# MIT-SPARK/Kimera-Semantics

Measured on NVIDIA H100. Metric: depth_frames_per_s, higher is better.
Workload: dtype f32

## Files before the change

### kimera_semantics_b200/csrc/ksg_api.cu

```cuda
#include <cuda_runtime.h>
#include <cub/cub.cuh>

#include <algorithm>
#include <climits>
#include <cmath>
#include <cstdio>
#include <cstdlib>
#include <cstring>
#include <memory>
#include <numeric>
#include <string>
#include <type_traits>
#include <unordered_map>
#include <unordered_set>
#include <utility>
#include <vector>

#include "../../include/ksg.h"
#include "ksg_kernels.cuh"
#include "ksg_chain.cuh"
#include "ksg_hot.cuh"
#include "ksg_bundle_order.cuh"
#include "ksg_fast.cuh"
#include "ksg_fast3.cuh"
// ... 154 lines not shown
  int frame_stamp = 0;
  int64_t num_blocks = 0;
  int64_t last_blocks_touched = 0;

  int cap_points = 0;
  float4 *pt_pC = nullptr, *pt_pG = nullptr;
  uint8_t *pt_label = nullptr, *pt_flags = nullptr;
  uint32_t* pt_color = nullptr;
  uint64_t* pt_key = nullptr;
  uint8_t* flags8 = nullptr;
  int* pix_list = nullptr;
  int* point_of_seq = nullptr;
  uint32_t *sq_keys = nullptr, *sq_keys_out = nullptr;
  uint32_t *iota = nullptr;

  int *start_next = nullptr, *start_min = nullptr, *start_max = nullptr;
  uint32_t *start_table = nullptr;
  int *s_base = nullptr, *s_visits = nullptr;
  uint32_t *s_hmin = nullptr, *s_hmax = nullptr;
  uint8_t *clear_ff = nullptr, *clear_00 = nullptr;
  uint64_t set_offset = 0;
  int64_t reset_counter = 0;
  int* cast_seq = nullptr;
  float4* ray_param = nullptr;
  uint8_t *ray_label = nullptr, *ray_flags = nullptr;
  uint32_t* ray_color = nullptr;
  int* nsteps = nullptr;
  RayState* ray_state = nullptr;
  long long* ext_off = nullptr;
  Obs3 o3{};

  uint64_t* ks_sorted = nullptr;
  uint32_t* seq_sorted = nullptr;
  int *bstart = nullptr, *bundle_f = nullptr;
  float *hist = nullptr, *tmp = nullptr, *tmp4 = nullptr;
// ... 27 lines not shown
  uint8_t* cub_temp = nullptr;
  size_t cub_temp_bytes = 0;

  uint8_t* h_stage = nullptr;
  size_t h_stage_bytes = 0;
  uint8_t* d_in = nullptr;
  size_t d_in_bytes = 0;

  uint8_t* d_exp = nullptr;
  size_t d_exp_bytes = 0;
  int* d_exp_slots = nullptr;
  int exp_slots_cap = 0;

  FastCounters* d_fc = nullptr;
  FastCounters* h_fc = nullptr;
  int *blk_cnt = nullptr, *blk_off = nullptr, *warp_cnt = nullptr, *warp_off = nullptr, *seq_of_i = nullptr;
  uint32_t* keys32 = nullptr;
  int *tile_cnt = nullptr, *tile_slot = nullptr;
  TileDesc* tile_list = nullptr;
  FastTile* fast_tiles = nullptr;
  FastItem* fast_items = nullptr;
  int item_cap = 0;
  int solve_grid = 0, group_grid = 0, fast_apply_grid = 0;
  int solve_threads = 0;
  RayRec* rayrec = nullptr;
  int* wl = nullptr;
  int *mixed_list = nullptr, *m_list = nullptr, *blk_run = nullptr;
  VoxelUpdate *d_log_head = nullptr, *h_log_head = nullptr;
  float *d_log_prior = nullptr, *h_log_prior = nullptr;
  int log_cap = 0;
  int64_t merged_log_count = 0;
// ... 77 lines not shown
    why = "unknown merged_bundle_order"; return KSG_ERR_INVALID_ARGUMENT; }
  if (c->hot_voxel_mode < 0 || c->hot_voxel_mode > 2) { why = "unknown hot_voxel_mode"; return KSG_ERR_INVALID_ARGUMENT; }
  return KSG_OK;
}

__global__ void k_iota(uint32_t* p, int n) { const int i = blockIdx.x * blockDim.x + threadIdx.x; if (i < n) p[i] = (uint32_t)i; }

int reset_map(ksg_integrator* h, cudaStream_t s) {
  KSG_CUDA(cudaMemsetAsync(h->map.ht_keys, 0xFF, sizeof(uint64_t) * h->ht_cap, s));
  KSG_CUDA(cudaMemsetAsync(h->map.ht_slot, 0xFF, sizeof(int) * h->ht_cap, s));
  KSG_CUDA(cudaMemsetAsync(h->map.touched_stamp, 0, sizeof(int) * h->ht_cap, s));
  KSG_CUDA(cudaMemsetAsync(h->d_cnt, 0, sizeof(Counters), s));
  if (h->start_table) KSG_CUDA(cudaMemsetAsync(h->start_table, 0xFF, sizeof(uint32_t) * kSetSize, s));
  if (h->o3.table) KSG_CUDA(cudaMemsetAsync(h->o3.table, 0xFF, sizeof(uint32_t) * kSetSize, s));
  if (h->d_fc) KSG_CUDA(cudaMemsetAsync(h->d_fc, 0, sizeof(FastCounters), s));
  if (h->o3.stamp_max) {
    KSG_CUDA(cudaMemsetAsync(h->o3.stamp_max, 0x00, sizeof(uint64_t) * kSetSize, s));
    KSG_CUDA(cudaMemsetAsync(h->o3.stamp_min, 0xFF, sizeof(uint64_t) * kSetSize, s));
  }
  if (h->wl) KSG_CUDA(cudaMemsetAsync(h->wl, 0, sizeof(int) * (size_t)h->cap_points, s));
  if (h->tile_cnt) KSG_CUDA(cudaMemsetAsync(h->tile_cnt, 0, sizeof(int) * (size_t)h->ht_cap * h->dc.tiles_per_block, s));
  h->n_pend = 0; h->n_stash = 0;
  std::memset(h->h_cnt_base, 0, 2 * sizeof(Counters));
  h->set_offset = 0;
  h->reset_counter = 0;
  h->num_blocks = 0;
  h->frame_stamp = 0;
  h->last_blocks_touched = 0;
  h->deferred_status = 0;
  h->merged_log_count = 0;
// ... 174 lines not shown
      h->set_offset = 0;
      KSG_CUDA(cudaMemsetAsync(h->start_table, 0xFF, sizeof(uint32_t) * kSetSize, s));
      KSG_CUDA(cudaMemsetAsync(h->o3.table, 0xFF, sizeof(uint32_t) * kSetSize, s));
    }
  }
  return KSG_OK;
}

int integrate_fast(ksg_integrator* h, const InputDesc& in, const FrameIn& fin, const Xform& T, int cap, cudaStream_t s,
                   ksg_frame_stats* stats) {
  const bool sorted = h->cfg.integration_order_mode == KSG_ORDER_SORTED;
  { const int rcs = advance_sets(h, s); if (rcs) return rcs; }
  FastFrame f{};
  f.cfg = h->dc; f.T = T; f.in = fin; f.in.pix_list = nullptr; f.in.point_of_seq = nullptr;
  f.luts = h->d_luts; f.cnt = h->d_cnt; f.fc = h->d_fc; f.map = h->map;
  f.sb = StartBuf{h->start_next, h->start_min, h->start_max, h->start_table};
  f.set_offset = h->set_offset;
  f.capacity = cap;
  f.n_count_blocks = (cap + kCountBlock - 1) / kCountBlock;
  f.vec_ok = in.d_depth ? (((uintptr_t)in.d_depth % 16 == 0 && (uintptr_t)in.d_label_img % 4 == 0) ? 1 : 0) : 0;
  f.frame_stamp = h->frame_stamp;
  f.profile = (h->profiling && !h->profile_marks_only) ? 1 : 0;
  f.prof_marks = h->profiling ? 1 : 0;
  f.seq_of_i = sorted ? h->seq_of_i : nullptr;
  f.block_cnt = h->blk_cnt; f.block_off = h->blk_off; f.warp_cnt = h->warp_cnt; f.warp_off = h->warp_off;
  f.pt_pG = h->pt_pG; f.pt_label = h->pt_label; f.pt_flags = h->pt_flags; f.pt_color = h->pt_color; f.pt_key = h->pt_key;
  f.cast_flag = h->flags8;
  f.cast_seq = h->cast_seq; f.ray_param = h->ray_param; f.ray_label = h->ray_label; f.ray_flags = h->ray_flags; f.ray_color = h->ray_color;
  f.ray_state = h->ray_state; f.ext_off = h->ext_off;
  f.rec_cap = h->rec_cap; f.keys = h->keys32;
  f.tile_cnt = h->tile_cnt; f.tile_slot = h->tile_slot; f.tile_list = h->tile_list; f.tile_cap = h->tile_cap;
  f.o3 = h->o3;
  f.rayrec = h->rayrec; f.blk_run = h->blk_run;
  f.wl_listed = h->wl;
  f.wl_list[0] = h->wl + h->cap_points; f.wl_list[1] = h->wl + 2 * (size_t)h->cap_points;
  f.log_head = h->d_log_head; f.log_prior = h->d_log_prior; f.log_cap = h->log_cap;
  f.s_base = h->s_base; f.s_hmin = h->s_hmin; f.s_hmax = h->s_hmax; f.s_visits = h->s_visits;
  f.mixed_list = h->mixed_list; f.m_list = h->m_list;

  if (h->profiling) {
    cudaEventRecord(h->ev[0], s);
    KSG_CUDA(cudaMemsetAsync(h->d_fc->dbg, 0, sizeof(h->d_fc->dbg), s));
  }
  KSG_CUDA(cudaMemsetAsync(h->clear_ff, 0xFF, (size_t)kSetSize * 16, s));
  KSG_CUDA(cudaMemsetAsync(h->clear_00, 0x00, (size_t)kSetSize * 13, s));
  KSG_CUDA(cudaMemsetAsync(h->start_min, 0x7F, sizeof(int) * kSetSize, s));
  const int B = 256;
  ++h->n_launches;
  if (in.d_depth) k_fast_count<<<f.n_count_blocks, 256, 0, s>>>(f);
  else k_fast_reset<<<1, 1, 0, s>>>(f);
  if (sorted) {
    h->n_launches += 3;
    if (in.d_depth) k_fast_sqnorm<<<f.n_count_blocks, 256, 0, s>>>(f, h->sq_keys);
    else k_fast_sqnorm_points<<<grid_for(cap, B), B, 0, s>>>(f, h->sq_keys);
    k_fast_pad_keys<<<grid_for(cap, B), B, 0, s>>>(h->d_cnt, cap, h->sq_keys);
    size_t tb = h->cub_temp_bytes;
    ++h->n_libcalls;
    KSG_CUDA(cub::DeviceRadixSort::SortPairs(h->cub_temp, tb, h->sq_keys, h->sq_keys_out, h->iota, (uint32_t*)h->point_of_seq, cap, 0, 32, s));
    k_fast_invert_perm<<<grid_for(cap, B), B, 0, s>>>(h->d_cnt, (const uint32_t*)h->point_of_seq, h->seq_of_i);
  }
  ++h->n_launches;
  if (in.d_depth) k_fast_classify<true><<<f.n_count_blocks, 256, 0, s>>>(f);
  else k_fast_classify<false><<<grid_for(cap, B), B, 0, s>>>(f);
  ++h->n_launches;
  k_fast_start_eval3<<<(cap + kEvalBlock - 1) / kEvalBlock, kEvalBlock, 0, s>>>(f);
  if (h->profiling) cudaEventRecord(h->ev[1], s);
  {
    int max_sweeps = h->cap_points + 2;
    void* args[] = {(void*)&f, (void*)&max_sweeps};
    ++h->n_launches;
    KSG_CUDA(cudaLaunchCooperativeKernel((const void*)k_fast_solve3, dim3(h->solve_grid), dim3(h->solve_threads), args,
                                         (size_t)h->solve_smem, s));
  }
  if (h->profiling) cudaEventRecord(h->ev[2], s);
  {
    ApplySrc src{};
    src.param = h->ray_param; src.label = h->ray_label; src.color = h->ray_color; src.tmp = nullptr;
    h->n_launches += 2;
    k_fast_group<<<h->group_grid, kGroupThreads, 0, s>>>(f, h->fast_items, h->fast_tiles, h->item_cap);
    with_nch(h->apply_nch, [&](auto nch) {
// ... 500 lines not shown
  KSG_CUDA(res.device(&h->map.pool, (size_t)dc.block_stride * (size_t)cfg->max_blocks));
  KSG_CUDA(res.device(&h->d_cnt, 1));
  KSG_CUDA(res.pinned(&h->h_cnt_base, 2));
  std::memset(h->h_cnt_base, 0, 2 * sizeof(Counters));
  h->h_cnt = h->h_cnt_base;
  for (int i = 0; i < 2; ++i) {
    KSG_CUDA(res.event(&h->ev_frame_s[i], cudaEventDisableTiming));
    KSG_CUDA(res.event(&h->ev_copy[i], cudaEventDisableTiming));
    KSG_CUDA(res.event(&h->ev_free[i], cudaEventDisableTiming));
  }
  KSG_CUDA(res.stream(&h->copy_stream));

  const size_t N = (size_t)cfg->max_points;
  h->cap_points = cfg->max_points;
  const bool fast = cfg->integrator_type == KSG_INTEGRATOR_FAST;
  KSG_CUDA(res.device(&h->pt_pC, N)); KSG_CUDA(res.device(&h->pt_pG, N));
  KSG_CUDA(res.device(&h->pt_label, N)); KSG_CUDA(res.device(&h->pt_flags, N));
  KSG_CUDA(res.device(&h->pt_color, N)); KSG_CUDA(res.device(&h->pt_key, N));
  KSG_CUDA(res.device(&h->flags8, 2 * N));
  KSG_CUDA(res.device(&h->pix_list, N));
  KSG_CUDA(res.device(&h->iota, N));
  k_iota<<<grid_for((long long)N, 256), 256>>>(h->iota, (int)N);
  if (cfg->integration_order_mode == KSG_ORDER_SORTED) {
    KSG_CUDA(res.device(&h->point_of_seq, N)); KSG_CUDA(res.device(&h->sq_keys, N)); KSG_CUDA(res.device(&h->sq_keys_out, N));
  }
  KSG_CUDA(res.device(&h->ray_param, N)); KSG_CUDA(res.device(&h->ray_flags, N)); KSG_CUDA(res.device(&h->nsteps, N));
  long long rec_cap = cfg->max_updates > 0 ? cfg->max_updates : (fast ? std::max<long long>(4ll << 20, 64ll * (long long)N) : (64ll << 20));
  if (fast) {
    KSG_CUDA(res.device(&h->start_next, N)); KSG_CUDA(res.device(&h->start_table, kSetSize));
    KSG_CUDA(res.device(&h->clear_ff, (size_t)kSetSize * 16));
    KSG_CUDA(res.device(&h->clear_00, (size_t)kSetSize * 13));
    h->s_base = (int*)h->clear_ff; h->start_max = h->s_base + kSetSize; h->s_hmin = (uint32_t*)(h->start_max + kSetSize);
    h->o3.head = (int*)(h->clear_ff + (size_t)kSetSize * 12);
    h->o3.slot_cnt = (int*)h->clear_00;
    h->s_hmax = (uint32_t*)(h->clear_00 + (size_t)kSetSize * 5); h->s_visits = (int*)(h->clear_00 + (size_t)kSetSize * 9);
    KSG_CUDA(res.device(&h->start_min, kSetSize));
    KSG_CUDA(res.device(&h->cast_seq, N));
    KSG_CUDA(res.device(&h->ray_label, N)); KSG_CUDA(res.device(&h->ray_color, N));
    KSG_CUDA(res.device(&h->ray_state, N)); KSG_CUDA(res.device(&h->ext_off, N * kExtSegs));
    long long ext = cfg->max_ray_steps > 0 ? cfg->max_ray_steps : std::max<long long>(16ll << 20, 64ll * (long long)N);
    Obs3& o3 = h->o3;
    o3.ext_base = (long long)N * kH0;
    o3.cand_cap = o3.ext_base + ext;
    if (o3.cand_cap >= 0x7FFFFFFFll) { o3.cand_cap = 0x7FFFFFFEll; }
    KSG_CUDA(res.device(&o3.cand, (size_t)o3.cand_cap));
    o3.ovf_cap = (int)std::min<long long>(std::max<long long>(1ll << 20, 4ll * (long long)N), 1ll << 28);
    KSG_CUDA(res.device(&o3.ovf, (size_t)o3.ovf_cap));
    KSG_CUDA(res.device(&o3.bkt, (size_t)kSetSize * kBkt3));
    KSG_CUDA(res.device(&o3.stamp_max, 2 * (size_t)kSetSize)); o3.stamp_min = o3.stamp_max + kSetSize;
    KSG_CUDA(res.device(&o3.table, kSetSize));
    KSG_CUDA(res.device(&h->rayrec, N));
// ... 104 lines not shown
    KSG_CUDA(cudaFuncSetAttribute(k_tile_apply<true, 1, true>, cudaFuncAttributeMaxDynamicSharedMemorySize, h->apply_smem));
    rc = for_each_tma_nch([&](auto tma, auto nch) -> int {
      KSG_CUDA(cudaFuncSetAttribute(k_tile_apply<decltype(tma)::value, decltype(nch)::value>, cudaFuncAttributeMaxDynamicSharedMemorySize,
                                    h->apply_smem));
      return KSG_OK;
    });
    if (rc) return rc;
  }
  if (fast) {
    KSG_CUDA(res.device(&h->d_fc, 1));
    KSG_CUDA(cudaMemset(h->d_fc, 0, sizeof(FastCounters)));
    KSG_CUDA(res.pinned(&h->h_fc_base, 2));
    std::memset(h->h_fc_base, 0, 2 * sizeof(FastCounters));
    h->h_fc = h->h_fc_base;
    KSG_CUDA(res.device(&h->blk_cnt, N / kCountBlock + 2)); KSG_CUDA(res.device(&h->blk_off, N / kCountBlock + 2));
    KSG_CUDA(res.device(&h->warp_cnt, N / 32 + 64)); KSG_CUDA(res.device(&h->warp_off, N / 32 + 64));
    if (cfg->integration_order_mode == KSG_ORDER_SORTED) KSG_CUDA(res.device(&h->seq_of_i, N));
    KSG_CUDA(res.device(&h->keys32, (size_t)rec_cap));
    const size_t n_tk = (size_t)h->ht_cap * dc.tiles_per_block;
    KSG_CUDA(res.device(&h->tile_cnt, n_tk)); KSG_CUDA(res.device(&h->tile_slot, n_tk));
    KSG_CUDA(cudaMemset(h->tile_cnt, 0, sizeof(int) * n_tk));
    KSG_CUDA(res.device(&h->tile_list, (size_t)h->tile_cap));
    {
      int per_sm = 0;
      h->solve_threads = knobs.solve_threads;
      h->solve_smem = (int)(sizeof(int) * kSortPerWarp * (h->solve_threads / 32));
      KSG_CUDA(cudaFuncSetAttribute(k_fast_solve3, cudaFuncAttributeMaxDynamicSharedMemorySize, h->solve_smem));
      KSG_CUDA(cudaOccupancyMaxActiveBlocksPerMultiprocessor(&per_sm, k_fast_solve3, h->solve_threads, (size_t)h->solve_smem));
      int coop = 0;
      cudaDeviceGetAttribute(&coop, cudaDevAttrCooperativeLaunch, h->device);
      if (!coop || per_sm <= 0) return h->fail(KSG_ERR_NO_DEVICE, "this device cannot run the fast integrator's observed-set solver "
// ... 1368 lines not shown
```

### kimera_semantics_b200/csrc/ksg_fast.cuh

```cuda
#pragma once
#include "ksg_kernels.cuh"

namespace ksg {

static constexpr int kCountBlock = 1024;
static constexpr int kEvalBlock = 512;
static constexpr int kSolveThreads = 1024;
static constexpr int kFastKeyCap = 4096;
static constexpr int kGroupThreads = 512;
static constexpr int kFastApplyThreads = 256;
static constexpr int kRecVoxMax = 1 << kRecVoxBits;
static constexpr int kTimelineSlots = 64;

struct FastCounters {
  unsigned int ticket_count, ticket_eval;
  unsigned int gridbar;
  int sweep_base;
  int sweeps_last;
  int tile_cursor;
  int n_tile_list;
  int pool_base;
  unsigned long long rec_cursor;
  int ovf_count;
  int n_mixed;
  int m_cursor;
  int log_count;
  int item_cursor;
  int wl_claim[4];
  int wl_count[4];
  long long timeline[kTimelineSlots];
  long long dbg[16];
};

struct TileDesc { uint32_t tk; int n; long long off; };
struct __align__(16) FastTile { long long off; int slot, tile, bx, by, bz, pad; };
struct __align__(16) FastItem { int tile, vox, lo, len; };

struct VoxelUpdate { int bx, by, bz; uint32_t lin_label; float dist, wgt; uint32_t rgba, srgba; };

struct StartBuf {
  int* next;
  int* smin;
  int* smax;
  const uint32_t* table;
};

struct Cand;
struct OvfEnt;
struct RayRec;
struct Obs3 {
  Cand* cand;
  long long ext_base, cand_cap;
  int* slot_cnt;
  uint64_t* bkt;
  int* head;
  OvfEnt* ovf;
  int ovf_cap;
  uint64_t* stamp_max;
  uint64_t* stamp_min;
// ... 6 lines not shown
  FrameIn in;
  const Luts* luts;
  Counters* cnt;
  FastCounters* fc;
  MapRef map;
  StartBuf sb;
  uint64_t set_offset;
  int capacity;
  int n_count_blocks;
  int vec_ok;
  int frame_stamp;
  int profile;
  int prof_marks;
  const int* seq_of_i;
  int* block_cnt; int* block_off;
  int* warp_cnt; int* warp_off;
  float4* pt_pG; uint8_t* pt_label; uint8_t* pt_flags; uint32_t* pt_color; uint64_t* pt_key; uint8_t* cast_flag;
  int* cast_seq; float4* ray_param; uint8_t* ray_label; uint8_t* ray_flags; uint32_t* ray_color;
  RayState* ray_state; long long* ext_off;
  long long rec_cap;
  uint32_t* keys;
  int* tile_cnt;
  int* tile_slot;
  TileDesc* tile_list; long long tile_cap;
  Obs3 o3;
  RayRec* rayrec;
  int* blk_run;
  int* wl_listed;
  int* wl_list[2];
  VoxelUpdate* log_head; float* log_prior; int log_cap;
  int* s_visits;
  uint32_t *s_hmin, *s_hmax;
  int* s_base;
  int* mixed_list;
  int* m_list;
};

__device__ __forceinline__ int inv_mixed_index(int i, int n) {
  const int groups = n / 1024;
  if (groups * 1024 <= i) return i;
  return (i % 1024) * groups + i / 1024;
}

__device__ __forceinline__ int block_scan_array(const int* a, int* out, int n) {
  __shared__ int s_w[32];
  __shared__ int s_total;
  const int tid = threadIdx.x, lane = tid & 31, wid = tid >> 5;
  const int nthreads = blockDim.x, nwarps = nthreads >> 5;
  const int per = (((n + nthreads - 1) / nthreads) + 3) & ~3;
  const int i0 = min(n, tid * per), i1 = min(n, i0 + per);
  int local = 0;
  {
    int i = i0;
    for (; i + 4 <= i1; i += 4) { const int4 v = __ldcg((const int4*)(a + i)); local += v.x + v.y + v.z + v.w; }
    for (; i < i1; ++i) local += __ldcg(&a[i]);
  }
  int incl = local;
  for (int o = 1; o < 32; o <<= 1) { const int v = __shfl_up_sync(0xffffffffu, incl, o); if (lane >= o) incl += v; }
  if (lane == 31) s_w[wid] = incl;
  __syncthreads();
  if (tid == 0) { int t = 0; for (int w = 0; w < nwarps; ++w) { const int v = s_w[w]; s_w[w] = t; t += v; } s_total = t; }
  __syncthreads();
  int run = s_w[wid] + incl - local;
  {
    int i = i0;
    for (; i + 4 <= i1; i += 4) {
      const int4 v = __ldcg((const int4*)(a + i));
      int4 r; r.x = run; r.y = run + v.x; r.z = r.y + v.y; r.w = r.z + v.z;
      *(int4*)(out + i) = r;
      run = r.w + v.w;
    }
    for (; i < i1; ++i) { const int v = __ldcg(&a[i]); out[i] = run; run += v; }
  }
  return s_total;
}

__device__ __forceinline__ void load_depth4(const float* __restrict__ depth, int p0, int P, int vec_ok, float d[4], int& npx) {
  npx = P - p0; if (npx > 4) npx = 4; if (npx < 0) npx = 0;
  if (npx == 4 && vec_ok) { const float4 v = __ldg((const float4*)(depth + p0)); d[0] = v.x; d[1] = v.y; d[2] = v.z; d[3] = v.w; }
  else { for (int k = 0; k < 4; ++k) d[k] = (k < npx) ? __ldg(depth + p0 + k) : 0.0f; }
}
__device__ __forceinline__ int first_finite_index(const FastFrame& f, const float d[4], int npx) {
  __shared__ int s_w[8];
  const int tid = threadIdx.x, lane = tid & 31, wid = tid >> 5;
  int c = 0;
  for (int k = 0; k < 4; ++k) c += (k < npx && isfinite(d[k])) ? 1 : 0;
  int incl = c;
// ... 19 lines not shown
  __syncthreads();
  if (tid == 0) {
    int t = 0; for (int w = 0; w < 8; ++w) t += s_w[w];
    __stcg(&f.block_cnt[blockIdx.x], t);
    __threadfence();
    s_last = (atomicAdd(&f.fc->ticket_count, 1u) == (unsigned)(f.n_count_blocks - 1));
  }
  __syncthreads();
  if (!s_last) return;
  __threadfence();
  const int total = block_scan_array(f.block_cnt, f.block_off, f.n_count_blocks);
  if (tid == 0) { frame_counters_reset(f.cnt, total); f.fc->ticket_count = 0; }
}
__global__ void k_fast_reset(FastFrame f) { frame_counters_reset(f.cnt, f.capacity); }

__device__ __forceinline__ void fast_classify_one(const FastFrame& f, int seq, F3 pC, uint8_t label, uint32_t color, bool& valid) {
  const DevCfg& cfg = f.cfg;
  bool clearing;
  point_test(cfg, f.in.freespace, f.cnt, pC, label, valid, clearing);
  if (f.luts->dynamic_label[label]) valid = false;
  const float w = point_weight(cfg, pC);
  const F3 pG = xform_apply(f.T, pC);
  f.pt_pG[seq] = make_float4(pG.x, pG.y, pG.z, w);
  f.pt_label[seq] = label;
  f.pt_color[seq] = color;
  f.pt_flags[seq] = (valid ? 1 : 0) | (clearing ? 2 : 0);
  uint64_t key = ~0ull;
  if (valid) {
    const F3 sc = mul(pG, cfg.start_inv);
    if (!index_in_range(sc)) set_err(f.cnt, 5);
    const I3 g = grid_index(pG, cfg.start_inv);
    key = (uint64_t)index_hash(g) + f.set_offset;
    const uint32_t slot = (uint32_t)key & kSetMask, hi = (uint32_t)(key >> kSetBits);
    f.sb.next[seq] = atomicAdd(&f.s_visits[slot], 1);
    atomicMin(&f.sb.smin[slot], seq);
    atomicMax(&f.sb.smax[slot], seq);
    atomicMin(&f.s_hmin[slot], hi);
    atomicMax(&f.s_hmax[slot], hi);
  }
  f.pt_key[seq] = key;
}

template <bool DEPTH>
__global__ void __launch_bounds__(256) k_fast_classify(FastFrame f) {
  const int tid = threadIdx.x, lane = tid & 31;
  const int n = f.cnt->n_points;
  int nvalid = 0;
  if (DEPTH) {
    const int p0 = blockIdx.x * kCountBlock + tid * 4;
    float d[4]; int npx;
    load_depth4(f.in.depth, p0, f.capacity, f.vec_ok, d, npx);
    uint8_t lab[4] = {0, 0, 0, 0};
    if (npx == 4 && f.vec_ok) { const uchar4 v = __ldg((const uchar4*)(f.in.label_img + p0)); lab[0] = v.x; lab[1] = v.y; lab[2] = v.z; lab[3] = v.w; }
    else { for (int k = 0; k < npx; ++k) lab[k] = __ldg(f.in.label_img + p0 + k); }
    int i = first_finite_index(f, d, npx);
    for (int k = 0; k < npx; ++k) {
      if (!isfinite(d[k])) continue;
      const int pix = p0 + k;
      const F3 pC = backproject(f.in, pix, d[k]);
      const int seq = f.seq_of_i ? f.seq_of_i[i] : inv_mixed_index(i, n);
      bool valid;
      fast_classify_one(f, seq, pC, lab[k], f.in.color_img ? f.in.color_img[pix] : f.luts->label_rgba[lab[k]], valid);
      nvalid += valid ? 1 : 0;
      ++i;
    }
  } else {
    const int i = blockIdx.x * blockDim.x + tid;
    if (i < n) {
      F3 pC;
      uint32_t color;
      uint8_t label;
      point_input(f.in, f.luts, i, pC, color, label);
      const int seq = f.seq_of_i ? f.seq_of_i[i] : inv_mixed_index(i, n);
      bool valid;
      fast_classify_one(f, seq, pC, label, color, valid);
      nvalid = valid ? 1 : 0;
    }
  }
  for (int o = 16; o > 0; o >>= 1) nvalid += __shfl_down_sync(0xffffffffu, nvalid, o);
  if (lane == 0 && nvalid) atomicAdd(&f.cnt->n_valid, nvalid);
}

__global__ void __launch_bounds__(256) k_fast_sqnorm(FastFrame f, uint32_t* __restrict__ keys) {
  const int p0 = blockIdx.x * kCountBlock + threadIdx.x * 4;
  float d[4]; int npx;
  load_depth4(f.in.depth, p0, f.capacity, f.vec_ok, d, npx);
  int i = first_finite_index(f, d, npx);
  for (int k = 0; k < npx; ++k) {
    if (!isfinite(d[k])) continue;
    const F3 pC = backproject(f.in, p0 + k, d[k]);
    keys[i++] = __float_as_uint(dot3(pC, pC));
  }
// ... 1 lines not shown
__global__ void k_fast_sqnorm_points(FastFrame f, uint32_t* __restrict__ keys) {
  const int i = blockIdx.x * blockDim.x + threadIdx.x;
  if (i >= f.capacity) return;
  const F3 pC = f3(f.in.xyz[3 * i], f.in.xyz[3 * i + 1], f.in.xyz[3 * i + 2]);
  keys[i] = __float_as_uint(dot3(pC, pC));
}
__global__ void k_fast_pad_keys(const Counters* cnt, int capacity, uint32_t* __restrict__ keys) {
  const int i = blockIdx.x * blockDim.x + threadIdx.x;
  if (i < capacity && i >= cnt->n_points) keys[i] = 0xFFFFFFFFu;
}
__global__ void k_fast_invert_perm(const Counters* cnt, const uint32_t* __restrict__ point_of_seq, int* __restrict__ seq_of_i) {
  const int s = blockIdx.x * blockDim.x + threadIdx.x;
  if (s < cnt->n_points) seq_of_i[point_of_seq[s]] = s;
}

__global__ void __launch_bounds__(kEvalBlock) k_fast_start_eval3(FastFrame f) {
  const int seq = blockIdx.x * kEvalBlock + threadIdx.x;
  const int lane = threadIdx.x & 31;
  const StartBuf& sb = f.sb;
  uint8_t cast = 0;
  if (seq < f.cnt->n_points) {
    const uint64_t v = f.pt_key[seq];
    if (v != ~0ull) {
      const uint32_t slot = (uint32_t)v & kSetMask, hi = (uint32_t)(v >> kSetBits);
      if (sb.smin[slot] == seq) {
        cast = sb.table[slot] != hi;
        ((uint32_t*)sb.table)[slot] = (uint32_t)(f.pt_key[sb.smax[slot]] >> kSetBits);
        if (f.s_hmin[slot] != f.s_hmax[slot]) {
          f.s_base[slot] = atomicAdd(&f.fc->m_cursor, f.s_visits[slot]);
          f.mixed_list[atomicAdd(&f.fc->n_mixed, 1)] = (int)slot;
        }
      }
    }
  }
  if (seq < f.capacity) f.cast_flag[seq] = cast;
  const unsigned m = __ballot_sync(0xffffffffu, cast != 0);
  if (lane == 0) __stcg(&f.warp_cnt[seq >> 5], __popc(m));
  if (blockIdx.x == 0 && threadIdx.x == 0) f.fc->gridbar = 0;
}

__device__ __forceinline__ void warp_sort_i32(int* a, int n, int lane) {
  int n2 = 1;
  while (n2 < n) n2 <<= 1;
  const int half = n2 >> 1;
  for (int k = 2; k <= n2; k <<= 1) {
    const int hk = k >> 1;
    for (int t = lane; t < half; t += 32) {
      const int blk = t / hk, o = t - blk * hk;
      const int i = blk * k + o, p = blk * k + (k - 1 - o);
      if (p < n) { const int x = a[i], y = a[p]; if (x > y) { a[i] = y; a[p] = x; } }
    }
    __syncwarp();
    for (int j = k >> 2; j > 0; j >>= 1) {
// ... 269 lines not shown
```

### kimera_semantics_b200/csrc/ksg_fast3.cuh

```cuda
#pragma once
#include <cuda/atomic>
#include "ksg_fast.cuh"

namespace ksg {

struct __align__(16) Cand { uint64_t vkey; int pos; int tog; };
struct __align__(16) OvfEnt { uint64_t order_perf; uint32_t hi; int next; };
struct __align__(16) RayRec { int H, L, nsteps, eval_sweep; };
static constexpr int kBkt3 = 32;
static constexpr int kOvfPending = -2;
static constexpr int kSortPerWarp = 1024;

__device__ __forceinline__ Cand ld_cand(const Cand* p) {
  const int4 v = __ldcg((const int4*)p);
  Cand c; c.vkey = ((uint64_t)(uint32_t)v.y << 32) | (uint32_t)v.x; c.pos = v.z; c.tog = v.w;
  return c;
}
__device__ __forceinline__ void st_cand(Cand* p, uint64_t vkey, int pos, int tog) {
  __stcg((int4*)p, make_int4((int)(uint32_t)vkey, (int)(uint32_t)(vkey >> 32), pos, tog));
}
__device__ __forceinline__ void st_cand_state(Cand* p, int pos, int tog) { __stcg((int2*)p + 1, make_int2(pos, tog)); }
__device__ __forceinline__ uint64_t cand_value(uint64_t vkey, uint64_t offset) { return (uint64_t)index_hash(unpack_key(vkey)) + offset; }
__device__ __forceinline__ uint64_t make_entry(bool on, uint64_t order, uint64_t v) { return (on ? kEntPerf : 0ull) | (order << 13) | (v >> kSetBits); }
__device__ __forceinline__ long long cand_index3(const Obs3& o, const long long* ext_off, int r, int s) {
// ... 222 lines not shown
  if (s < kH0) { s0 = 0; blen = kH0; return; }
  const int k = 31 - __clz(s >> 4);
  const int seg = kH0 << k;
  if (seg <= kWin) { s0 = seg; blen = seg; }
  else { s0 = seg + ((s - seg) & ~(kWin - 1)); blen = kWin; }
}

__device__ __forceinline__ void fast3_ray_setup(const FastFrame& f, int r, int n_cast) {
  const DevCfg& cfg = f.cfg;
  const Obs3& o = f.o3;
  int h = 0;
  const long long t_begin = f.profile ? clock64() : 0;
  long long t_ins = 0;
  if (r < n_cast) {
    const int seq = f.cast_seq[r];
    const float4 p = f.pt_pG[seq];
    const uint8_t fl = f.pt_flags[seq];
    f.ray_param[r] = p;
    f.ray_label[r] = f.pt_label[seq];
    f.ray_flags[r] = fl;
    f.ray_color[r] = f.pt_color[seq];
    if (f.profile) dbg_max(f, 12, clock64() - t_begin);
    Dda d;
    raycaster_init(d, f3(f.T.tx, f.T.ty, f.T.tz), f3(p.x, p.y, p.z), (fl & 2) != 0, cfg.carving != 0, cfg.max_ray, cfg.vsi, cfg.tp.trunc,
                   false);
    int n = d.length_in_steps + 1;
    if (!d.in_range || n >= (1 << kOrderStepBits)) { set_err(f.cnt, 5); n = 0; }
    if (f.profile) dbg_max(f, 13, clock64() - t_begin);
    h = n < kH0 ? n : kH0;
    const int l0 = h < cfg.maxc ? h : cfg.maxc;
    for (int s = 0; s < h; ++s) {
      const I3 g = dda_next(d);
      if (!key_in_range(g)) { set_err(f.cnt, 5); h = s; break; }
      const uint64_t vkey = pack_key(g);
      const long long ci = (long long)r * kH0 + s;
      int pos = -2;
// ... 250 lines not shown

__global__ void __launch_bounds__(kSolveThreads, 1) k_fast_solve3(FastFrame f, int max_sweeps) {
  unsigned int epoch = 0;
  unsigned int* bar = &f.fc->gridbar;
  const int lane = threadIdx.x & 31;
  const int gtid0 = (((threadIdx.x >> 5) * gridDim.x + blockIdx.x) << 5) | lane;
  const int gthreads = gridDim.x * blockDim.x;
  Counters* cnt = f.cnt;
  const int n_points = cnt->n_points;
  int tl = 0;
  timeline_mark(f, tl++);
  extern __shared__ int s_sort[];
  const int n_mixed = ((volatile int*)&f.fc->n_mixed)[0];
  if (n_mixed > 0) {
    if (gtid0 == 0) f.fc->wl_claim[0] = 0;
    for (int seq = gtid0; seq < n_points; seq += gthreads) {
      const uint64_t v = f.pt_key[seq];
      if (v == ~0ull) continue;
      const uint32_t slot = (uint32_t)v & kSetMask;
      if (f.s_hmin[slot] != f.s_hmax[slot]) f.m_list[f.s_base[slot] + f.sb.next[seq]] = seq;
    }
    solve_barrier(bar, epoch);
    timeline_mark(f, 57);
    const int warps_total = gthreads >> 5;
    int* scratch = s_sort + (threadIdx.x >> 5) * kSortPerWarp;
    for (int mi = (threadIdx.x >> 5) * gridDim.x + blockIdx.x; mi < n_mixed;) {
      const int slot = f.mixed_list[mi];
      const int n = __ldcg(&f.s_visits[slot]);
      int* seg = f.m_list + __ldcg(&f.s_base[slot]);
      int* a = seg;
      if (n <= kSortPerWarp) { for (int i = lane; i < n; i += 32) scratch[i] = __ldcg(&seg[i]); a = scratch; }
      __syncwarp();
      warp_sort_i32(a, n, lane);
      for (int i = 1 + lane; i < n; i += 32) {
        const int pa = a[i - 1], pb = a[i];
        if (f.pt_key[pa] != f.pt_key[pb]) { f.cast_flag[pb] = 1; atomicAdd(&f.warp_cnt[pb >> 5], 1); }
      }
      __syncwarp();
      if (f.profile && lane == 0) { dbg_max(f, 8, n); dbg_add(f, 9, n); }
      int next = 0;
      if (lane == 0) next = warps_total + atomicAdd(&f.fc->wl_claim[0], 1);
      mi = __shfl_sync(0xffffffffu, next, 0);
    }
    solve_barrier(bar, epoch);
    timeline_mark(f, 58);
  }
  if (blockIdx.x == 0) {
    const int n_warps32 = (f.capacity + 31) >> 5;
    const int total = block_scan_array(f.warp_cnt, f.warp_off, n_warps32);
    if (threadIdx.x == 0) cnt->n_cast = total;
  }
  solve_barrier(bar, epoch);
  timeline_mark(f, 59);
  const int n_cast = ((volatile int*)&cnt->n_cast)[0];
  for (int base = (gtid0 & ~31); base < n_points; base += gthreads) {
    const int seq = base + lane;
    const bool c = seq < n_points && __ldcg(&f.cast_flag[seq]) != 0;
    const unsigned m = __ballot_sync(0xffffffffu, c);
    if (c) f.cast_seq[__ldcg(&f.warp_off[seq >> 5]) + __popc(m & ((1u << lane) - 1u))] = seq;
  }
  const int sweep_base0 = ((volatile int*)&f.fc->sweep_base)[0];
  if (gtid0 == 0) for (int k = 0; k < 4; ++k) { f.fc->wl_claim[k] = 0; f.fc->wl_count[k] = 0; }
  solve_barrier(bar, epoch);
  timeline_mark(f, tl++);
  for (int r0 = (gtid0 & ~31); r0 < n_cast; r0 += gthreads) fast3_ray_setup(f, r0 + lane, n_cast);
  solve_barrier(bar, epoch);
  timeline_mark(f, tl++);
  int sweep = (sweep_base0 + 4) & ~3;
  bool converged = n_cast == 0;
  int it = 0;
  while (!converged && it < max_sweeps) {
    ++it;
    ++sweep;
    fast3_sweep(f, sweep, it, (WarpDdaScratch*)(s_sort + (threadIdx.x >> 5) * kSortPerWarp));
// ... 47 lines not shown
  const bool ok2 = ((volatile int*)&cnt->err)[0] == 0 && !failed;
  if (!failed) fast3_walk_performed<2>(f, ((volatile int*)&cnt->n_cast)[0], ok2 ? n_tiles : 0, gtid);
  if (gtid == 0) {
    int add = n_new;
    if (pool_base + add > f.map.max_blocks) add = f.map.max_blocks - pool_base;
    if (ok) cnt->pool_count = pool_base + (add > 0 ? add : 0);
    cnt->n_tiles = ok2 ? n_tiles : 0;
    cnt->n_records = ((volatile unsigned long long*)&f.fc->rec_cursor)[0];
    f.fc->tile_cursor = 0;
    f.fc->n_tile_list = 0;
    f.fc->rec_cursor = 0;
    f.fc->ovf_count = 0;
    if (f.profile) { f.fc->dbg[10] = ((volatile int*)&f.fc->n_mixed)[0]; f.fc->dbg[11] = ((volatile int*)&cnt->n_cast)[0]; }
    f.fc->n_mixed = 0;
    f.fc->m_cursor = 0;
    f.fc->log_count = 0;
  }
  timeline_mark(f, tl++);
}

}
```

Measured before the change: 2217.

## Pack start-slot state into records and evaluate only touched slots

Replaces the separate per-slot arrays (next, min, max, hmin, hmax, visits) with a packed 16-byte StartRec and a list of touched slots. The per-point evaluation kernel becomes a slot-driven pass over only the touched slots, and records reset themselves after use, so the large per-frame memsets of the set tables go away. Cast flags become a bitmask with a popcount scan, and per-point world position, label and colour are no longer stored; they are recomputed from the pixel for the points that cast rays. The cost is extra recomputation in ray setup, atomics aggregated within each thread's four pixels, and more complex bookkeeping for the mixed-slot path.

```diff
diff --git a/kimera_semantics_b200/csrc/ksg_api.cu b/kimera_semantics_b200/csrc/ksg_api.cu
--- a/kimera_semantics_b200/csrc/ksg_api.cu
+++ b/kimera_semantics_b200/csrc/ksg_api.cu
@@ -192,11 +192,9 @@
   uint32_t *sq_keys = nullptr, *sq_keys_out = nullptr;
   uint32_t *iota = nullptr;
 
-  int *start_next = nullptr, *start_min = nullptr, *start_max = nullptr;
+  StartRec* start_rec = nullptr;
   uint32_t *start_table = nullptr;
-  int *s_base = nullptr, *s_visits = nullptr;
-  uint32_t *s_hmin = nullptr, *s_hmax = nullptr;
-  uint8_t *clear_ff = nullptr, *clear_00 = nullptr;
+  int* start_touched = nullptr;
   uint64_t set_offset = 0;
   int64_t reset_counter = 0;
   int* cast_seq = nullptr;
@@ -254,7 +252,8 @@
 
   FastCounters* d_fc = nullptr;
   FastCounters* h_fc = nullptr;
-  int *blk_cnt = nullptr, *blk_off = nullptr, *warp_cnt = nullptr, *warp_off = nullptr, *seq_of_i = nullptr;
+  int *blk_cnt = nullptr, *blk_off = nullptr, *warp_off = nullptr, *seq_of_i = nullptr;
+  uint32_t* cast_bits = nullptr;
   uint32_t* keys32 = nullptr;
   int *tile_cnt = nullptr, *tile_slot = nullptr;
   TileDesc* tile_list = nullptr;
@@ -362,6 +361,11 @@
   if (h->start_table) KSG_CUDA(cudaMemsetAsync(h->start_table, 0xFF, sizeof(uint32_t) * kSetSize, s));
   if (h->o3.table) KSG_CUDA(cudaMemsetAsync(h->o3.table, 0xFF, sizeof(uint32_t) * kSetSize, s));
   if (h->d_fc) KSG_CUDA(cudaMemsetAsync(h->d_fc, 0, sizeof(FastCounters), s));
+  if (h->start_rec) {
+    KSG_CUDA(cudaMemset2DAsync(&h->start_rec->first, sizeof(StartRec), 0xFF, 2 * sizeof(uint32_t), kSetSize, s));
+    KSG_CUDA(cudaMemset2DAsync(&h->start_rec->hmax, sizeof(StartRec), 0x00, 2 * sizeof(uint32_t), kSetSize, s));
+  }
+  if (h->cast_bits) KSG_CUDA(cudaMemsetAsync(h->cast_bits, 0, sizeof(uint32_t) * ((size_t)h->cap_points / 32 + 64), s));
   if (h->o3.stamp_max) {
     KSG_CUDA(cudaMemsetAsync(h->o3.stamp_max, 0x00, sizeof(uint64_t) * kSetSize, s));
     KSG_CUDA(cudaMemsetAsync(h->o3.stamp_min, 0xFF, sizeof(uint64_t) * kSetSize, s));
@@ -566,7 +570,7 @@
   FastFrame f{};
   f.cfg = h->dc; f.T = T; f.in = fin; f.in.pix_list = nullptr; f.in.point_of_seq = nullptr;
   f.luts = h->d_luts; f.cnt = h->d_cnt; f.fc = h->d_fc; f.map = h->map;
-  f.sb = StartBuf{h->start_next, h->start_min, h->start_max, h->start_table};
+  f.sb = StartBuf{h->start_rec, h->start_table, h->start_touched, sorted ? h->point_of_seq : nullptr};
   f.set_offset = h->set_offset;
   f.capacity = cap;
   f.n_count_blocks = (cap + kCountBlock - 1) / kCountBlock;
@@ -575,9 +579,8 @@
   f.profile = (h->profiling && !h->profile_marks_only) ? 1 : 0;
   f.prof_marks = h->profiling ? 1 : 0;
   f.seq_of_i = sorted ? h->seq_of_i : nullptr;
-  f.block_cnt = h->blk_cnt; f.block_off = h->blk_off; f.warp_cnt = h->warp_cnt; f.warp_off = h->warp_off;
-  f.pt_pG = h->pt_pG; f.pt_label = h->pt_label; f.pt_flags = h->pt_flags; f.pt_color = h->pt_color; f.pt_key = h->pt_key;
-  f.cast_flag = h->flags8;
+  f.block_cnt = h->blk_cnt; f.block_off = h->blk_off; f.cast_bits = h->cast_bits; f.warp_off = h->warp_off;
+  f.pt_key = h->pt_key; f.pt_pix = h->pix_list;
   f.cast_seq = h->cast_seq; f.ray_param = h->ray_param; f.ray_label = h->ray_label; f.ray_flags = h->ray_flags; f.ray_color = h->ray_color;
   f.ray_state = h->ray_state; f.ext_off = h->ext_off;
   f.rec_cap = h->rec_cap; f.keys = h->keys32;
@@ -587,16 +590,14 @@
   f.wl_listed = h->wl;
   f.wl_list[0] = h->wl + h->cap_points; f.wl_list[1] = h->wl + 2 * (size_t)h->cap_points;
   f.log_head = h->d_log_head; f.log_prior = h->d_log_prior; f.log_cap = h->log_cap;
-  f.s_base = h->s_base; f.s_hmin = h->s_hmin; f.s_hmax = h->s_hmax; f.s_visits = h->s_visits;
   f.mixed_list = h->mixed_list; f.m_list = h->m_list;
 
   if (h->profiling) {
     cudaEventRecord(h->ev[0], s);
     KSG_CUDA(cudaMemsetAsync(h->d_fc->dbg, 0, sizeof(h->d_fc->dbg), s));
   }
-  KSG_CUDA(cudaMemsetAsync(h->clear_ff, 0xFF, (size_t)kSetSize * 16, s));
-  KSG_CUDA(cudaMemsetAsync(h->clear_00, 0x00, (size_t)kSetSize * 13, s));
-  KSG_CUDA(cudaMemsetAsync(h->start_min, 0x7F, sizeof(int) * kSetSize, s));
+  KSG_CUDA(cudaMemsetAsync(h->o3.head, 0xFF, sizeof(int) * kSetSize, s));
+  KSG_CUDA(cudaMemsetAsync(h->o3.slot_cnt, 0x00, sizeof(int) * kSetSize, s));
   const int B = 256;
   ++h->n_launches;
   if (in.d_depth) k_fast_count<<<f.n_count_blocks, 256, 0, s>>>(f);
@@ -615,7 +616,7 @@
   if (in.d_depth) k_fast_classify<true><<<f.n_count_blocks, 256, 0, s>>>(f);
   else k_fast_classify<false><<<grid_for(cap, B), B, 0, s>>>(f);
   ++h->n_launches;
-  k_fast_start_eval3<<<(cap + kEvalBlock - 1) / kEvalBlock, kEvalBlock, 0, s>>>(f);
+  k_fast_start_slots<<<std::min(grid_for(cap, B), 4 * h->sm_count), B, 0, s>>>(f);
   if (h->profiling) cudaEventRecord(h->ev[1], s);
   {
     int max_sweeps = h->cap_points + 2;
@@ -1146,9 +1147,12 @@
   const size_t N = (size_t)cfg->max_points;
   h->cap_points = cfg->max_points;
   const bool fast = cfg->integrator_type == KSG_INTEGRATOR_FAST;
-  KSG_CUDA(res.device(&h->pt_pC, N)); KSG_CUDA(res.device(&h->pt_pG, N));
-  KSG_CUDA(res.device(&h->pt_label, N)); KSG_CUDA(res.device(&h->pt_flags, N));
-  KSG_CUDA(res.device(&h->pt_color, N)); KSG_CUDA(res.device(&h->pt_key, N));
+  if (!fast) {
+    KSG_CUDA(res.device(&h->pt_pC, N)); KSG_CUDA(res.device(&h->pt_pG, N));
+    KSG_CUDA(res.device(&h->pt_label, N)); KSG_CUDA(res.device(&h->pt_flags, N));
+    KSG_CUDA(res.device(&h->pt_color, N));
+  }
+  KSG_CUDA(res.device(&h->pt_key, N));
   KSG_CUDA(res.device(&h->flags8, 2 * N));
   KSG_CUDA(res.device(&h->pix_list, N));
   KSG_CUDA(res.device(&h->iota, N));
@@ -1159,14 +1163,9 @@
   KSG_CUDA(res.device(&h->ray_param, N)); KSG_CUDA(res.device(&h->ray_flags, N)); KSG_CUDA(res.device(&h->nsteps, N));
   long long rec_cap = cfg->max_updates > 0 ? cfg->max_updates : (fast ? std::max<long long>(4ll << 20, 64ll * (long long)N) : (64ll << 20));
   if (fast) {
-    KSG_CUDA(res.device(&h->start_next, N)); KSG_CUDA(res.device(&h->start_table, kSetSize));
-    KSG_CUDA(res.device(&h->clear_ff, (size_t)kSetSize * 16));
-    KSG_CUDA(res.device(&h->clear_00, (size_t)kSetSize * 13));
-    h->s_base = (int*)h->clear_ff; h->start_max = h->s_base + kSetSize; h->s_hmin = (uint32_t*)(h->start_max + kSetSize);
-    h->o3.head = (int*)(h->clear_ff + (size_t)kSetSize * 12);
-    h->o3.slot_cnt = (int*)h->clear_00;
-    h->s_hmax = (uint32_t*)(h->clear_00 + (size_t)kSetSize * 5); h->s_visits = (int*)(h->clear_00 + (size_t)kSetSize * 9);
-    KSG_CUDA(res.device(&h->start_min, kSetSize));
+    KSG_CUDA(res.device(&h->start_rec, kSetSize)); KSG_CUDA(res.device(&h->start_table, kSetSize));
+    KSG_CUDA(res.device(&h->start_touched, N));
+    KSG_CUDA(res.device(&h->o3.head, kSetSize)); KSG_CUDA(res.device(&h->o3.slot_cnt, kSetSize));
     KSG_CUDA(res.device(&h->cast_seq, N));
     KSG_CUDA(res.device(&h->ray_label, N)); KSG_CUDA(res.device(&h->ray_color, N));
     KSG_CUDA(res.device(&h->ray_state, N)); KSG_CUDA(res.device(&h->ext_off, N * kExtSegs));
@@ -1301,7 +1300,7 @@
     std::memset(h->h_fc_base, 0, 2 * sizeof(FastCounters));
     h->h_fc = h->h_fc_base;
     KSG_CUDA(res.device(&h->blk_cnt, N / kCountBlock + 2)); KSG_CUDA(res.device(&h->blk_off, N / kCountBlock + 2));
-    KSG_CUDA(res.device(&h->warp_cnt, N / 32 + 64)); KSG_CUDA(res.device(&h->warp_off, N / 32 + 64));
+    KSG_CUDA(res.device(&h->cast_bits, N / 32 + 64)); KSG_CUDA(res.device(&h->warp_off, N / 32 + 64));
     if (cfg->integration_order_mode == KSG_ORDER_SORTED) KSG_CUDA(res.device(&h->seq_of_i, N));
     KSG_CUDA(res.device(&h->keys32, (size_t)rec_cap));
     const size_t n_tk = (size_t)h->ht_cap * dc.tiles_per_block;
diff --git a/kimera_semantics_b200/csrc/ksg_fast.cuh b/kimera_semantics_b200/csrc/ksg_fast.cuh
--- a/kimera_semantics_b200/csrc/ksg_fast.cuh
+++ b/kimera_semantics_b200/csrc/ksg_fast.cuh
@@ -4,7 +4,6 @@
 namespace ksg {
 
 static constexpr int kCountBlock = 1024;
-static constexpr int kEvalBlock = 512;
 static constexpr int kSolveThreads = 1024;
 static constexpr int kFastKeyCap = 4096;
 static constexpr int kGroupThreads = 512;
@@ -13,7 +12,7 @@
 static constexpr int kTimelineSlots = 64;
 
 struct FastCounters {
-  unsigned int ticket_count, ticket_eval;
+  unsigned int ticket_count;
   unsigned int gridbar;
   int sweep_base;
   int sweeps_last;
@@ -22,6 +21,7 @@
   int pool_base;
   unsigned long long rec_cursor;
   int ovf_count;
+  unsigned long long n_touched;
   int n_mixed;
   int m_cursor;
   int log_count;
@@ -38,11 +38,17 @@
 
 struct VoxelUpdate { int bx, by, bz; uint32_t lin_label; float dist, wgt; uint32_t rgba, srgba; };
 
+struct __align__(16) StartRec {
+  uint32_t first;
+  uint32_t hmin, hmax;
+  uint32_t visits;
+};
+__device__ __forceinline__ uint4 start_rec_empty() { return make_uint4(~0u, ~0u, 0u, 0u); }
 struct StartBuf {
-  int* next;
-  int* smin;
-  int* smax;
-  const uint32_t* table;
+  StartRec* rec;
+  uint32_t* table;
+  int* touched;
+  const int* i_of_seq;
 };
 
 struct Cand;
@@ -79,8 +85,9 @@
   int prof_marks;
   const int* seq_of_i;
   int* block_cnt; int* block_off;
-  int* warp_cnt; int* warp_off;
-  float4* pt_pG; uint8_t* pt_label; uint8_t* pt_flags; uint32_t* pt_color; uint64_t* pt_key; uint8_t* cast_flag;
+  uint32_t* cast_bits;
+  int* warp_off;
+  uint64_t* pt_key; int* pt_pix;
   int* cast_seq; float4* ray_param; uint8_t* ray_label; uint8_t* ray_flags; uint32_t* ray_color;
   RayState* ray_state; long long* ext_off;
   long long rec_cap;
@@ -94,9 +101,6 @@
   int* wl_listed;
   int* wl_list[2];
   VoxelUpdate* log_head; float* log_prior; int log_cap;
-  int* s_visits;
-  uint32_t *s_hmin, *s_hmax;
-  int* s_base;
   int* mixed_list;
   int* m_list;
 };
@@ -107,7 +111,9 @@
   return (i % 1024) * groups + i / 1024;
 }
 
+template <bool POPC = false>
 __device__ __forceinline__ int block_scan_array(const int* a, int* out, int n) {
+  auto val = [](int x) { return POPC ? __popc(x) : x; };
   __shared__ int s_w[32];
   __shared__ int s_total;
   const int tid = threadIdx.x, lane = tid & 31, wid = tid >> 5;
@@ -117,8 +123,8 @@
   int local = 0;
   {
     int i = i0;
-    for (; i + 4 <= i1; i += 4) { const int4 v = __ldcg((const int4*)(a + i)); local += v.x + v.y + v.z + v.w; }
-    for (; i < i1; ++i) local += __ldcg(&a[i]);
+    for (; i + 4 <= i1; i += 4) { const int4 v = __ldcg((const int4*)(a + i)); local += val(v.x) + val(v.y) + val(v.z) + val(v.w); }
+    for (; i < i1; ++i) local += val(__ldcg(&a[i]));
   }
   int incl = local;
   for (int o = 1; o < 32; o <<= 1) { const int v = __shfl_up_sync(0xffffffffu, incl, o); if (lane >= o) incl += v; }
@@ -131,11 +137,11 @@
     int i = i0;
     for (; i + 4 <= i1; i += 4) {
       const int4 v = __ldcg((const int4*)(a + i));
-      int4 r; r.x = run; r.y = run + v.x; r.z = r.y + v.y; r.w = r.z + v.z;
+      int4 r; r.x = run; r.y = run + val(v.x); r.z = r.y + val(v.y); r.w = r.z + val(v.z);
       *(int4*)(out + i) = r;
-      run = r.w + v.w;
-    }
-    for (; i < i1; ++i) { const int v = __ldcg(&a[i]); out[i] = run; run += v; }
+      run = r.w + val(v.w);
+    }
+    for (; i < i1; ++i) { const int v = val(__ldcg(&a[i])); out[i] = run; run += v; }
   }
   return s_total;
 }
@@ -185,31 +191,69 @@
 }
 __global__ void k_fast_reset(FastFrame f) { frame_counters_reset(f.cnt, f.capacity); }
 
-__device__ __forceinline__ void fast_classify_one(const FastFrame& f, int seq, F3 pC, uint8_t label, uint32_t color, bool& valid) {
+struct FastPoint { F3 pG; float w; uint32_t color; uint8_t label; bool valid, clearing; };
+__device__ __forceinline__ FastPoint fast_point(const FastFrame& f, int pix, float d) {
   const DevCfg& cfg = f.cfg;
-  bool clearing;
-  point_test(cfg, f.in.freespace, f.cnt, pC, label, valid, clearing);
-  if (f.luts->dynamic_label[label]) valid = false;
-  const float w = point_weight(cfg, pC);
-  const F3 pG = xform_apply(f.T, pC);
-  f.pt_pG[seq] = make_float4(pG.x, pG.y, pG.z, w);
-  f.pt_label[seq] = label;
-  f.pt_color[seq] = color;
-  f.pt_flags[seq] = (valid ? 1 : 0) | (clearing ? 2 : 0);
-  uint64_t key = ~0ull;
-  if (valid) {
-    const F3 sc = mul(pG, cfg.start_inv);
-    if (!index_in_range(sc)) set_err(f.cnt, 5);
-    const I3 g = grid_index(pG, cfg.start_inv);
-    key = (uint64_t)index_hash(g) + f.set_offset;
-    const uint32_t slot = (uint32_t)key & kSetMask, hi = (uint32_t)(key >> kSetBits);
-    f.sb.next[seq] = atomicAdd(&f.s_visits[slot], 1);
-    atomicMin(&f.sb.smin[slot], seq);
-    atomicMax(&f.sb.smax[slot], seq);
-    atomicMin(&f.s_hmin[slot], hi);
-    atomicMax(&f.s_hmax[slot], hi);
-  }
-  f.pt_key[seq] = key;
+  FastPoint p;
+  F3 pC;
+  if (f.in.depth) {
+    pC = backproject(f.in, pix, d);
+    p.label = __ldg(f.in.label_img + pix);
+    p.color = f.in.color_img ? f.in.color_img[pix] : f.luts->label_rgba[p.label];
+  } else {
+    point_input(f.in, f.luts, pix, pC, p.color, p.label);
+  }
+  point_test(cfg, f.in.freespace, f.cnt, pC, p.label, p.valid, p.clearing);
+  if (f.luts->dynamic_label[p.label]) p.valid = false;
+  p.w = point_weight(cfg, pC);
+  p.pG = xform_apply(f.T, pC);
+  return p;
+}
+__device__ __forceinline__ uint64_t fast_start_key(const FastFrame& f, const FastPoint& p) {
+  if (!p.valid) return ~0ull;
+  const F3 sc = mul(p.pG, f.cfg.start_inv);
+  if (!index_in_range(sc)) set_err(f.cnt, 5);
+  const I3 g = grid_index(p.pG, f.cfg.start_inv);
+  return (uint64_t)index_hash(g) + f.set_offset;
+}
+
+template <int K>
+__device__ __forceinline__ void start_visits(const FastFrame& f, const uint64_t (&key)[K], const int (&seq)[K]) {
+  uint32_t slot[K];
+  bool head[K], fresh[K];
+  uint32_t prev = ~0u;
+#pragma unroll
+  for (int k = 0; k < K; ++k) {
+    slot[k] = (uint32_t)key[k] & kSetMask;
+    head[k] = key[k] != ~0ull && slot[k] != prev;
+    if (key[k] != ~0ull) prev = slot[k];
+    fresh[k] = false;
+  }
+#pragma unroll
+  for (int k = 0; k < K; ++k) {
+    if (!head[k]) continue;
+    uint32_t first = (uint32_t)seq[k], hmin = (uint32_t)(key[k] >> kSetBits), hmax = hmin, n = 1;
+    bool run = true;
+#pragma unroll
+    for (int j = k + 1; j < K; ++j) {
+      if (!run || key[j] == ~0ull) continue;
+      if (slot[j] != slot[k]) { run = false; continue; }
+      const uint32_t hi = (uint32_t)(key[j] >> kSetBits);
+      first = min(first, (uint32_t)seq[j]); hmin = min(hmin, hi); hmax = max(hmax, hi); ++n;
+    }
+    StartRec* r = &f.sb.rec[slot[k]];
+    atomicMin(&r->first, first);
+    atomicMin(&r->hmin, hmin);
+    atomicMax(&r->hmax, hmax);
+    fresh[k] = atomicAdd(&r->visits, n) == 0;
+  }
+  int n_fresh = 0;
+#pragma unroll
+  for (int k = 0; k < K; ++k) n_fresh += fresh[k] ? 1 : 0;
+  int at = (int)warp_alloc(&f.fc->n_touched, (unsigned long long)n_fresh);
+#pragma unroll
+  for (int k = 0; k < K; ++k)
+    if (fresh[k]) f.sb.touched[at++] = (int)slot[k];
 }
 
 template <bool DEPTH>
@@ -221,32 +265,35 @@
     const int p0 = blockIdx.x * kCountBlock + tid * 4;
     float d[4]; int npx;
     load_depth4(f.in.depth, p0, f.capacity, f.vec_ok, d, npx);
-    uint8_t lab[4] = {0, 0, 0, 0};
-    if (npx == 4 && f.vec_ok) { const uchar4 v = __ldg((const uchar4*)(f.in.label_img + p0)); lab[0] = v.x; lab[1] = v.y; lab[2] = v.z; lab[3] = v.w; }
-    else { for (int k = 0; k < npx; ++k) lab[k] = __ldg(f.in.label_img + p0 + k); }
     int i = first_finite_index(f, d, npx);
-    for (int k = 0; k < npx; ++k) {
-      if (!isfinite(d[k])) continue;
+    uint64_t key[4];
+    int seq[4];
+#pragma unroll
+    for (int k = 0; k < 4; ++k) {
+      key[k] = ~0ull; seq[k] = 0;
+      if (k >= npx || !isfinite(d[k])) continue;
       const int pix = p0 + k;
-      const F3 pC = backproject(f.in, pix, d[k]);
-      const int seq = f.seq_of_i ? f.seq_of_i[i] : inv_mixed_index(i, n);
-      bool valid;
-      fast_classify_one(f, seq, pC, lab[k], f.in.color_img ? f.in.color_img[pix] : f.luts->label_rgba[lab[k]], valid);
-      nvalid += valid ? 1 : 0;
+      const FastPoint p = fast_point(f, pix, d[k]);
+      seq[k] = f.seq_of_i ? f.seq_of_i[i] : inv_mixed_index(i, n);
+      key[k] = fast_start_key(f, p);
+      f.pt_key[i] = key[k];
+      f.pt_pix[i] = pix;
+      nvalid += p.valid ? 1 : 0;
       ++i;
     }
+    start_visits<4>(f, key, seq);
   } else {
     const int i = blockIdx.x * blockDim.x + tid;
+    uint64_t key[1] = {~0ull};
+    int seq[1] = {0};
     if (i < n) {
-      F3 pC;
-      uint32_t color;
-      uint8_t label;
-      point_input(f.in, f.luts, i, pC, color, label);
-      const int seq = f.seq_of_i ? f.seq_of_i[i] : inv_mixed_index(i, n);
-      bool valid;
-      fast_classify_one(f, seq, pC, label, color, valid);
-      nvalid = valid ? 1 : 0;
-    }
+      const FastPoint p = fast_point(f, i, 0.0f);
+      seq[0] = f.seq_of_i ? f.seq_of_i[i] : inv_mixed_index(i, n);
+      key[0] = fast_start_key(f, p);
+      f.pt_key[i] = key[0];
+      nvalid = p.valid ? 1 : 0;
+    }
+    start_visits<1>(f, key, seq);
   }
   for (int o = 16; o > 0; o >>= 1) nvalid += __shfl_down_sync(0xffffffffu, nvalid, o);
   if (lane == 0 && nvalid) atomicAdd(&f.cnt->n_valid, nvalid);
@@ -278,29 +325,22 @@
   if (s < cnt->n_points) seq_of_i[point_of_seq[s]] = s;
 }
 
-__global__ void __launch_bounds__(kEvalBlock) k_fast_start_eval3(FastFrame f) {
-  const int seq = blockIdx.x * kEvalBlock + threadIdx.x;
-  const int lane = threadIdx.x & 31;
-  const StartBuf& sb = f.sb;
-  uint8_t cast = 0;
-  if (seq < f.cnt->n_points) {
-    const uint64_t v = f.pt_key[seq];
-    if (v != ~0ull) {
-      const uint32_t slot = (uint32_t)v & kSetMask, hi = (uint32_t)(v >> kSetBits);
-      if (sb.smin[slot] == seq) {
-        cast = sb.table[slot] != hi;
-        ((uint32_t*)sb.table)[slot] = (uint32_t)(f.pt_key[sb.smax[slot]] >> kSetBits);
-        if (f.s_hmin[slot] != f.s_hmax[slot]) {
-          f.s_base[slot] = atomicAdd(&f.fc->m_cursor, f.s_visits[slot]);
-          f.mixed_list[atomicAdd(&f.fc->n_mixed, 1)] = (int)slot;
-        }
-      }
-    }
-  }
-  if (seq < f.capacity) f.cast_flag[seq] = cast;
-  const unsigned m = __ballot_sync(0xffffffffu, cast != 0);
-  if (lane == 0) __stcg(&f.warp_cnt[seq >> 5], __popc(m));
+__global__ void __launch_bounds__(256) k_fast_start_slots(FastFrame f) {
   if (blockIdx.x == 0 && threadIdx.x == 0) f.fc->gridbar = 0;
+  const int n = (int)f.fc->n_touched;
+  for (int t = blockIdx.x * blockDim.x + threadIdx.x; t < n; t += gridDim.x * blockDim.x) {
+    const uint32_t slot = (uint32_t)f.sb.touched[t];
+    StartRec* r = &f.sb.rec[slot];
+    const uint4 v = *(const uint4*)r;
+    if (v.y == v.z) {
+      if (f.sb.table[slot] != v.y) atomicOr(&f.cast_bits[v.x >> 5], 1u << (v.x & 31));
+      f.sb.table[slot] = v.y;
+      *(uint4*)r = start_rec_empty();
+    } else {
+      r->first = (uint32_t)atomicAdd(&f.fc->m_cursor, (int)v.w);
+      f.mixed_list[atomicAdd(&f.fc->n_mixed, 1)] = (int)slot;
+    }
+  }
 }
 
 __device__ __forceinline__ void warp_sort_i32(int* a, int n, int lane) {
diff --git a/kimera_semantics_b200/csrc/ksg_fast3.cuh b/kimera_semantics_b200/csrc/ksg_fast3.cuh
--- a/kimera_semantics_b200/csrc/ksg_fast3.cuh
+++ b/kimera_semantics_b200/csrc/ksg_fast3.cuh
@@ -260,12 +260,15 @@
   long long t_ins = 0;
   if (r < n_cast) {
     const int seq = f.cast_seq[r];
-    const float4 p = f.pt_pG[seq];
-    const uint8_t fl = f.pt_flags[seq];
+    const int i = f.sb.i_of_seq ? f.sb.i_of_seq[seq] : mixed_index(seq, __ldcg(&f.cnt->n_points));
+    const int pix = f.in.depth ? f.pt_pix[i] : i;
+    const FastPoint q = fast_point(f, pix, f.in.depth ? __ldg(f.in.depth + pix) : 0.0f);
+    const float4 p = make_float4(q.pG.x, q.pG.y, q.pG.z, q.w);
+    const uint8_t fl = (q.valid ? 1 : 0) | (q.clearing ? 2 : 0);
     f.ray_param[r] = p;
-    f.ray_label[r] = f.pt_label[seq];
+    f.ray_label[r] = q.label;
     f.ray_flags[r] = fl;
-    f.ray_color[r] = f.pt_color[seq];
+    f.ray_color[r] = q.color;
     if (f.profile) dbg_max(f, 12, clock64() - t_begin);
     Dda d;
     raycaster_init(d, f3(f.T.tx, f.T.ty, f.T.tz), f3(p.x, p.y, p.z), (fl & 2) != 0, cfg.carving != 0, cfg.max_ray, cfg.vsi, cfg.tp.trunc,
@@ -546,29 +549,37 @@
   const int n_mixed = ((volatile int*)&f.fc->n_mixed)[0];
   if (n_mixed > 0) {
     if (gtid0 == 0) f.fc->wl_claim[0] = 0;
-    for (int seq = gtid0; seq < n_points; seq += gthreads) {
-      const uint64_t v = f.pt_key[seq];
+    for (int i = gtid0; i < n_points; i += gthreads) {
+      const uint64_t v = __ldcg(&f.pt_key[i]);
       if (v == ~0ull) continue;
-      const uint32_t slot = (uint32_t)v & kSetMask;
-      if (f.s_hmin[slot] != f.s_hmax[slot]) f.m_list[f.s_base[slot] + f.sb.next[seq]] = seq;
+      StartRec* r = &f.sb.rec[(uint32_t)v & kSetMask];
+      if (__ldcg(&r->visits) != 0) f.m_list[atomicAdd(&r->first, 1u)] = f.seq_of_i ? f.seq_of_i[i] : inv_mixed_index(i, n_points);
     }
     solve_barrier(bar, epoch);
     timeline_mark(f, 57);
     const int warps_total = gthreads >> 5;
     int* scratch = s_sort + (threadIdx.x >> 5) * kSortPerWarp;
+    auto key_of_seq = [&](int seq) { return __ldcg(&f.pt_key[f.sb.i_of_seq ? f.sb.i_of_seq[seq] : mixed_index(seq, n_points)]); };
     for (int mi = (threadIdx.x >> 5) * gridDim.x + blockIdx.x; mi < n_mixed;) {
       const int slot = f.mixed_list[mi];
-      const int n = __ldcg(&f.s_visits[slot]);
-      int* seg = f.m_list + __ldcg(&f.s_base[slot]);
+      StartRec* rec = &f.sb.rec[slot];
+      const int n = (int)__ldcg(&rec->visits);
+      int* seg = f.m_list + ((int)__ldcg(&rec->first) - n);
       int* a = seg;
       if (n <= kSortPerWarp) { for (int i = lane; i < n; i += 32) scratch[i] = __ldcg(&seg[i]); a = scratch; }
       __syncwarp();
       warp_sort_i32(a, n, lane);
-      for (int i = 1 + lane; i < n; i += 32) {
-        const int pa = a[i - 1], pb = a[i];
-        if (f.pt_key[pa] != f.pt_key[pb]) { f.cast_flag[pb] = 1; atomicAdd(&f.warp_cnt[pb >> 5], 1); }
+      for (int i = lane; i < n; i += 32) {
+        const int sb = a[i];
+        const uint64_t kb = key_of_seq(sb);
+        const bool cast = i == 0 ? f.sb.table[slot] != (uint32_t)(kb >> kSetBits) : key_of_seq(a[i - 1]) != kb;
+        if (cast) atomicOr(&f.cast_bits[sb >> 5], 1u << (sb & 31));
       }
       __syncwarp();
+      if (lane == 0) {
+        f.sb.table[slot] = (uint32_t)(key_of_seq(a[n - 1]) >> kSetBits);
+        *(uint4*)rec = start_rec_empty();
+      }
       if (f.profile && lane == 0) { dbg_max(f, 8, n); dbg_add(f, 9, n); }
       int next = 0;
       if (lane == 0) next = warps_total + atomicAdd(&f.fc->wl_claim[0], 1);
@@ -577,19 +588,19 @@
     solve_barrier(bar, epoch);
     timeline_mark(f, 58);
   }
+  const int n_words = (f.capacity + 31) >> 5;
   if (blockIdx.x == 0) {
-    const int n_warps32 = (f.capacity + 31) >> 5;
-    const int total = block_scan_array(f.warp_cnt, f.warp_off, n_warps32);
+    const int total = block_scan_array<true>((const int*)f.cast_bits, f.warp_off, n_words);
     if (threadIdx.x == 0) cnt->n_cast = total;
   }
   solve_barrier(bar, epoch);
   timeline_mark(f, 59);
   const int n_cast = ((volatile int*)&cnt->n_cast)[0];
-  for (int base = (gtid0 & ~31); base < n_points; base += gthreads) {
-    const int seq = base + lane;
-    const bool c = seq < n_points && __ldcg(&f.cast_flag[seq]) != 0;
-    const unsigned m = __ballot_sync(0xffffffffu, c);
-    if (c) f.cast_seq[__ldcg(&f.warp_off[seq >> 5]) + __popc(m & ((1u << lane) - 1u))] = seq;
+  for (int w = gtid0; w < n_words; w += gthreads) {
+    uint32_t m = __ldcg(&f.cast_bits[w]);
+    if (m == 0u) continue;
+    f.cast_bits[w] = 0u;
+    for (int at = __ldcg(&f.warp_off[w]); m; m &= m - 1u) f.cast_seq[at++] = (w << 5) | (__ffs(m) - 1);
   }
   const int sweep_base0 = ((volatile int*)&f.fc->sweep_base)[0];
   if (gtid0 == 0) for (int k = 0; k < 4; ++k) { f.fc->wl_claim[k] = 0; f.fc->wl_count[k] = 0; }
@@ -667,6 +678,7 @@
     if (f.profile) { f.fc->dbg[10] = ((volatile int*)&f.fc->n_mixed)[0]; f.fc->dbg[11] = ((volatile int*)&cnt->n_cast)[0]; }
     f.fc->n_mixed = 0;
     f.fc->m_cursor = 0;
+    f.fc->n_touched = 0;
     f.fc->log_count = 0;
   }
   timeline_mark(f, tl++);
```

Measured after the change: 2514 (median of 6 runs). +13.4%, better.
